# Nikhil-Doye/voice-enabled-browser-automation

Measured on AMD Instinct MI355X. Metric: voice-to-intent p50 latency (ms) + ASR RTF; 10s utterance; Llama-3-8B brain, lower is better.
Workload: dtype bf16; 1 GPU; model=whisper-tiny + llama3-8b, global_batch=1, parallelism=dp1, budget_chars=512, hipgraph=True

## Files before the change

### csrc/bindings.cpp

```cpp
#include <mutex>
#include <string>

#include <torch/extension.h>
#include <ATen/hip/impl/HIPStreamMasqueradingAsCUDA.h>
#include <c10/core/DeviceGuard.h>

#include "kernels/vwa_kernels.h"

namespace {

using at::Tensor;
using OptTensor = c10::optional<Tensor>;
constexpr auto kBF16 = at::kBFloat16;
constexpr auto kF8 = at::kFloat8_e4m3fn;

hipStream_t cur_stream(const Tensor& t) {
  return c10::hip::getCurrentHIPStreamMasqueradingAsCUDA(t.device().index()).stream();
}

const uint16_t* bfp(const Tensor& t) { return reinterpret_cast<const uint16_t*>(t.data_ptr()); }
uint16_t* bfp_mut(const Tensor& t) { return reinterpret_cast<uint16_t*>(t.data_ptr()); }
const uint16_t* bfp_opt(const OptTensor& t) { return t.has_value() ? bfp(*t) : nullptr; }
uint16_t* bfp_mut_opt(const OptTensor& t) { return t.has_value() ? bfp_mut(*t) : nullptr; }
template <class T>
// ... 570 lines not shown

int chain_grid(const Tensor& a) {
  const char* e = std::getenv("VWA_CHAIN_GRID_DIV");
  const int div = e ? std::atoi(e) : 1, cus = device_cus(a);
  return div > 1 ? cus / div : cus;
}

void chain_schedule(ChainParams& cp) {
  cp.pre2 = 1;
  cp.next0 = 1;
  cp.xdma = 1;
  cp.osub = 1;
  cp.lds_item_req = 1;
  cp.lds_item2_req = 1;
  cp.attn_flag = 1;
  cp.xfirst = 1;
  cp.xwait = 1;
  cp.o_nt2 = 1;
  cp.d_nt2 = 1;
  cp.pre_mask = 8;
  cp.qkv_flags = 0;
  cp.kv_prefetch = 0;
  cp.attn_pre = 0;
  if (const char* e = std::getenv("VWA_CHAIN_SCHED")) {
    std::string s(e);
    size_t at = 0;
    while (at < s.size()) {
      const size_t comma = s.find(',', at), eq = s.find('=', at);
      const size_t end = comma == std::string::npos ? s.size() : comma;
      if (eq != std::string::npos && eq < end) {
        const std::string k = s.substr(at, eq - at);
        const int v = std::atoi(s.substr(eq + 1, end - eq - 1).c_str());
        if (k == "pre2") cp.pre2 = v;
        else if (k == "next0") cp.next0 = v;
        else if (k == "xdma") cp.xdma = v;
        else if (k == "osub") cp.osub = v;
        else if (k == "lds1") cp.lds_item_req = v;
        else if (k == "lds2") cp.lds_item2_req = v;
        else if (k == "aflag") cp.attn_flag = v;
        else if (k == "pre_mask") cp.pre_mask = v;
        else if (k == "pre_waves") cp.pre_waves = v;
        else if (k == "xfirst") cp.xfirst = v;
        else if (k == "xwait") cp.xwait = v;
        else if (k == "xw_late") cp.xw_late = v;
        else if (k == "poll_free") cp.poll_free = v;
        else if (k == "o_nt2") cp.o_nt2 = v;
        else if (k == "d_nt2") cp.d_nt2 = v;
        else if (k == "qkv_flags") cp.qkv_flags = v;
        else if (k == "kv_pf") cp.kv_prefetch = v;
        else if (k == "attn_pre") cp.attn_pre = v;
      }
      at = end + 1;
    }
  }
}

void set_resid(SkinnyParams& p, const Tensor& h) {
  p.Y = h.data_ptr();
  p.ldy = (int)h.stride(0);
  p.R = bfp(h);
  p.ldr = (int)h.stride(0);
}

void set_chain_sync(ChainParams& cp, const Tensor& a, const Tensor& bar, const Tensor& work, int64_t bar_mode) {
  check_vec(bar, a, at::kInt, 384, "bar");
  TORCH_CHECK(aligned(bar, 128), "bar must be 128-byte aligned");
  check_vec(work, a, at::kInt, 8192 + 4096 + 1, "work");
  cp.bar = reinterpret_cast<unsigned*>(bar.data_ptr<int>());
  cp.bar_mode = (int)bar_mode;
  cp.tickets = reinterpret_cast<unsigned*>(work.data_ptr<int>());
  cp.max_tiles = 8192;
  cp.part = reinterpret_cast<float*>(work.data_ptr<int>() + 8192);
  cp.part_floats = (int)(work.numel() - 8192);
// ... 84 lines not shown
                            n_kv_heads, head_dim, a_scale, a_n_splits, *a_part_o, *a_part_ml, *a_counters, att);
    TORCH_CHECK(a_n_splits > 1, "attention phase: the in-launch chunk merge needs n_splits > 1");
    cp.attn_g = (int)(n_q_heads / n_kv_heads);
    TORCH_CHECK(a_row_table.has_value(), "attention phase: a_row_table (per-row block tables) is required");
    TORCH_CHECK(a_block_size == 16, "attention phase: 16-token KV blocks (mq_attention.h FINE addressing)");
    const Tensor& rtab = *a_row_table;
    check_vec(rtab, h, at::kInt, 0, "a_row_table");
    TORCH_CHECK(rtab.dim() == 2 && rtab.size(0) >= M && rtab.size(1) <= 128 && rtab.size(1) % 2 == 0,
                "a_row_table must be int32 [>= rows, <= 128 (even)] contiguous");
    cp.attn.row_table = rtab.data_ptr<int>();
    cp.attn.rt_stride = (int)rtab.size(1);
    if (a_plan_mode) {
      TORCH_CHECK(a_plan_mode == 1 || a_plan_mode == 2, "a_plan_mode: 1 write, 2 read");
      TORCH_CHECK(a_plan.has_value(), "a_plan_mode needs a_plan");
      check_vec(*a_plan, h, at::kInt, (int64_t)chain_grid(h) * 16, "a_plan");
      cp.attn.plan = a_plan->data_ptr<int>();
      cp.attn.plan_mode = (int)a_plan_mode;
    }
  }
  int64_t lds = 0;
  Tensor desc = chain_upload(cp, h, lds);
  if (!desc.numel()) return {desc, 0};
  return {desc, lds | (cp.n >= 3 && cp.ph[2].xg ? (int64_t)1 << 24 : 0) | (cp.d_nt2 ? (int64_t)1 << 27 : 0) |
                    (s_o.has_value() ? (int64_t)1 << 25 : 0) | (cp.o_nt2 ? (int64_t)1 << 26 : 0)};
}

std::tuple<Tensor, int64_t> chain_make_seq(int64_t seq, std::vector<Tensor> X, std::vector<Tensor> W,
                                           std::vector<OptTensor> bias, std::vector<OptTensor> ln_c,
                                           std::vector<Tensor> Y, std::vector<int64_t> epi, double eps, int64_t n_heads,
                                           int64_t head_dim, OptTensor positions, OptTensor slots, OptTensor k_cache,
                                           OptTensor v_cache, Tensor bar, Tensor work, int64_t bar_mode, bool w_tiled) {
  const size_t n = X.size();
  TORCH_CHECK(n >= 2 && n <= (size_t)kChainMaxPhases && W.size() == n && bias.size() == n && ln_c.size() == n &&
                  Y.size() == n && epi.size() == n,
              "chain_make_seq: one X/W/bias/ln_c/Y/epi per phase");
  TORCH_CHECK(seq == 1 || seq == 2, "chain_make_seq: seq 1 (Whisper tail) or 2 (Whisper middle)");
  const Tensor& a = X[0];
  c10::DeviceGuard g(a.device());
  check_anchor(a, "X");
  ChainParams cp{};
  set_chain_sync(cp, a, bar, work, bar_mode);
  for (size_t i = 0; i < n; ++i) {
    check_gpu(X[i], a, kBF16, "X");
    SkinnyParams& p = cp.ph[i].p;
    p = base_params(X[i], "X", W[i], "W", bias[i], "bias", false, eps, c10::nullopt, w_tiled);
    cp.ph[i].epi = (int)epi[i];
// ... 556 lines not shown
```

### csrc/kernels/mq_attention.h

```cpp
#pragma once
#include "common.h"
#include "vwa_kernels.h"

namespace {
using namespace vwa;

typedef __attribute__((address_space(1))) const int gint;
VWA_DEVICE int64_t kv_offset(const KVView& kv, int seq, int kvh, int t) {
  const int blk = *(gint*)(kv.block_table + (int64_t)seq * kv.table_stride + t / kv.block_size);
  return (int64_t)blk * kv.stride_block + (int64_t)kvh * kv.stride_head + (int64_t)(t % kv.block_size) * kv.stride_tok;
}

VWA_DEVICE __amdgpu_buffer_rsrc_t rsrc_f32(float* p, int64_t n) {
  return __builtin_amdgcn_make_buffer_rsrc(p, (short)0, (int)(n * 4), 0x00020000);
}
VWA_DEVICE void st_sc1_f2(__amdgpu_buffer_rsrc_t r, int64_t idx, float a, float b) {
  __builtin_amdgcn_raw_buffer_store_b64(__builtin_bit_cast(u32x2, make_float2(a, b)), r, (int)(idx * 4), 0, 16);
}
VWA_DEVICE void st_sc1_f1(__amdgpu_buffer_rsrc_t r, int64_t idx, float a) {
  __builtin_amdgcn_raw_buffer_store_b32(__float_as_uint(a), r, (int)(idx * 4), 0, 16);
}
VWA_DEVICE float2 ld_sc1_f2(__amdgpu_buffer_rsrc_t r, int64_t idx) {
  return __builtin_bit_cast(float2, __builtin_amdgcn_raw_buffer_load_b64(r, (int)(idx * 4), 0, 16));
}
// ... 36 lines not shown
    __hip_atomic_store(gp(reinterpret_cast<unsigned long long*>(dst) + 1), (unsigned long long)v.z | ((unsigned long long)v.w << 32),
                       __ATOMIC_RELAXED, __HIP_MEMORY_SCOPE_AGENT);
  } else {
    *gp(reinterpret_cast<u32x4*>(dst)) = u32x4{v.x, v.y, v.z, v.w};
  }
}

template <int D, int NW>
struct MqLds {
  static constexpr int OWP = D + 4;
  static constexpr int vimg = 0;
  static constexpr int ow = NW * kMqStep * 256;
  static constexpr int mlw = ow + NW * kMqCols * OWP * 4;
  static constexpr int last = mlw + NW * kMqCols * 2 * 4;
  static constexpr int bytes = last + 16;
};

struct NoIdle {
  VWA_DEVICE void operator()() const {}
};
struct NoStamp {
  VWA_DEVICE void operator()(int) const {}
};

template <int D, int G, int NW, bool SC1OUT, bool DB = true, bool FINE = false, class OnIdle = NoIdle,
          class Stamp = NoStamp, class OnKv = NoIdle>
VWA_DEVICE bool mq_body(const DecodeAttnParams& p, unsigned char* lds, int grid, int bid, OnIdle on_idle = {},
                        int* n_items_out = nullptr, Stamp stamp = {}, unsigned long long* done = nullptr,
                        int* n_final_out = nullptr, OnKv on_kv = {}) {
  constexpr int kWv = NW;
  constexpr int kChunk = FINE ? kMqStep : NW * kMqStep;
  constexpr int RG = kMqCols / G;
  constexpr int NKS = D / 32;
  constexpr int NDT = D / 16;
  constexpr int NCH = D / 8;
  constexpr int NVL = kMqStep * NCH / 64;
  constexpr int OWP = D + 4;
  using L = MqLds<D, NW>;
  float* ow = reinterpret_cast<float*>(lds + L::ow);
  float* mlw = reinterpret_cast<float*>(lds + L::mlw);
  int& s_last = *reinterpret_cast<int*>(lds + L::last);

  const int nkv = p.n_kv_heads, nq = p.n_q_heads;
  const int lane = VWA_TX & 63, w = VWA_TX >> 6;
  const int n = lane & 15, g = lane >> 4;

  constexpr bool rowtab = FINE;
  const __amdgpu_buffer_rsrc_t r_rt = __builtin_amdgcn_make_buffer_rsrc(
      const_cast<int*>(p.row_table), (short)0, rowtab ? p.rows * p.rt_stride * 4 : 0, 0x00020000);
  int* s_meta = reinterpret_cast<int*>(lds + L::vimg);
  int2 rt[4];
  int ev = 0;
  bool plan = false;
  if constexpr (FINE) {
    if (p.plan_mode == 2) {
      const __amdgpu_buffer_rsrc_t r_pl = __builtin_amdgcn_make_buffer_rsrc(p.plan, (short)0, (bid + 1) * 64, 0x00020000);
      ev = (int)__builtin_amdgcn_raw_buffer_load_b32(r_pl, (bid * 16 + (lane & 15)) * 4, 0, 16);
#pragma unroll
      for (int r = 0; r < 4; ++r)
        rt[r] = __builtin_bit_cast(int2, __builtin_amdgcn_raw_buffer_load_b64(
                                             r_rt, 2 * lane < p.rt_stride ? (r * p.rt_stride + 2 * lane) * 4 : 0x7FFFFFF0, 0, 0));
      plan = __builtin_amdgcn_readlane(ev, 2) != 3 && __builtin_amdgcn_readlane(ev, 10) == p.rows;
    }
  }
  if (w == 0 && !plan) {
#pragma unroll
    for (int r = 0; r < 4; ++r)
      *reinterpret_cast<int2*>(s_meta + r * 128 + 2 * lane) = __builtin_bit_cast(
          int2, __builtin_amdgcn_raw_buffer_load_b64(
                    r_rt, 2 * lane < p.rt_stride ? (r * p.rt_stride + 2 * lane) * 4 : 0x7FFFFFF0, 0, 0));
    const __amdgpu_buffer_rsrc_t r_sid =
        __builtin_amdgcn_make_buffer_rsrc(const_cast<int*>(p.seq_ids), (short)0, p.rows * 4, 0x00020000);
    const __amdgpu_buffer_rsrc_t r_ctx =
        __builtin_amdgcn_make_buffer_rsrc(const_cast<int*>(p.ctx_lens), (short)0, p.rows * 4, 0x00020000);
    s_meta[512 + lane] = (int)__builtin_amdgcn_raw_buffer_load_b32(r_sid, lane * 4, 0, 0);
    s_meta[576 + lane] = (int)__builtin_amdgcn_raw_buffer_load_b32(r_ctx, lane * 4, 0, 0);
    if constexpr (!FINE) {
      const __amdgpu_buffer_rsrc_t r_sh =
// ... 19 lines not shown
  }
  const bool cascade = !FINE && P > 0 && n_real > 0 && p.n_splits > RG;
  unsigned long long run_starts = seq_starts;
  if (cascade) {
    const unsigned long long real = n_real >= 64 ? ~0ull : ((1ull << n_real) - 1ull);
    run_starts = 1ull | (n_real < p.rows ? (1ull << n_real) : 0ull) | (seq_starts & ~real);
  }
  const int run0 = 63 - __builtin_clzll(run_starts & ((2ull << lane) - 1ull));
  const unsigned long long leaders = __ballot(lane < p.rows && (lane - run0) % RG == 0);
  const int n_groups = __builtin_popcountll(leaders);
  const int my_rank = __builtin_popcountll(leaders & ((1ull << lane) - 1ull));
  static_assert(!FINE || NW == 8, "the FINE merge pairs two threads per (column, slice): 512 threads");
  const int tgt = FINE ? grid : max(1, grid / 2);
  const int n_pc = cascade ? max(1, min(p.n_splits - RG, tgt / max(1, n_groups * nkv) - RG)) : 0;
  const int n_eff = cascade ? n_pc + RG : max(1, min(FINE ? min(p.n_splits, 16) : p.n_splits, tgt / max(1, n_groups * nkv)));
  const int n_items = plan ? __builtin_amdgcn_readlane(ev, 0) : n_groups * nkv * n_eff;
  if (n_items_out) *n_items_out = n_items;
  if (n_final_out) *n_final_out = plan ? __builtin_amdgcn_readlane(ev, 1) : n_groups * nkv;
  stamp(17);
  const bool multi = n_items > grid;
  auto write_plan = [&](int st, int kvh, int r0, int nr, int kbeg, int kend, int nact, int slot, int c) {
    if (!FINE || p.plan_mode != 1 || w != 0) return;
    const int cr = __shfl(c, lane & 3, 64);
    const int i = lane & 15;
    const int v = i == 0 ? n_items : i == 1 ? n_groups * nkv : i == 2 ? (multi ? 3 : st) : i == 3 ? kvh : i == 4 ? r0
                : i == 5 ? nr : i == 6 ? kbeg : i == 7 ? kend : i == 8 ? nact : i == 9 ? slot : i == 10 ? p.rows
                : i == 11 ? 0 : cr;
    if (lane < 16) p.plan[bid * 16 + i] = v;
  };
  if (bid >= n_items) {
    write_plan(0, 0, 0, 0, 0, 0, 0, 0, 0);
    on_idle();
    return true;
  }

  auto publish = [&]() {
    if (done == nullptr) return;
    asm volatile("s_waitcnt vmcnt(0)" ::: "memory");
    __syncthreads();
    if (VWA_TX == 0) __hip_atomic_fetch_add(gp(done), 1ull, __ATOMIC_RELAXED, __HIP_MEMORY_SCOPE_AGENT);
  };
  for (int item = bid; item < n_items; item += grid) {
  if (item == bid) stamp(18);
  int kvh, r0, nr, CL, kbeg, kend, nact, slot, kv_seq, ctx_n;
  const int rho = n / G;
  if (plan) {
    if (__builtin_amdgcn_readlane(ev, 2) != 1) continue;
    kvh = __builtin_amdgcn_readlane(ev, 3);
    r0 = __builtin_amdgcn_readlane(ev, 4);
    nr = __builtin_amdgcn_readlane(ev, 5);
// ... 85 lines not shown
  auto make_qf = [&]() {
    const float qs = p.scale * 1.4426950408889634f;
    const int64_t qo = (int64_t)(r0 + min(rho, nr - 1)) * p.ldq + (kvh * G + n % G) * D + 8 * g;
    const __amdgpu_buffer_rsrc_t r_q = __builtin_amdgcn_make_buffer_rsrc(
        const_cast<u16*>(p.q), (short)0, FINE ? (int)((int64_t)p.rows * p.ldq * 2) : 0, 0x00020000);
#pragma unroll
    for (int ks = 0; ks < NKS; ++ks) {
      float f[8];
      if constexpr (FINE) {
        const u32x4 v = __builtin_amdgcn_raw_buffer_load_b128(r_q, (int)((qo + 32 * ks) * 2), 0, 16);
        unpack8(make_uint4(v.x, v.y, v.z, v.w), f);
      } else {
        unpack8(ld128(p.q + qo + 32 * ks), f);
      }
#pragma unroll
      for (int j = 0; j < 8; ++j) f[j] = rho < nr ? f[j] * qs : 0.f;
      qf[ks] = as_bf16x8(pack8(f));
    }
  };
  if constexpr (DB) {
    make_qf();
    if (item == bid) stamp(10);
  }
  const int2 rtr = r0 == 0 ? rt[0] : r0 == 1 ? rt[1] : r0 == 2 ? rt[2] : rt[3];

  auto load_step = [&](int kb, uint4 (&kr)[2][NKS], uint4 (&vr)[NVL]) {
    int64_t ko[2], vo[NVL];
    auto offsets = [&](auto off) {
#pragma unroll
      for (int t = 0; t < 2; ++t) ko[t] = off(min(kb + 8 * (n >> 2) + 4 * t + (n & 3), kmax));
#pragma unroll
      for (int i = 0; i < NVL; ++i) vo[i] = off(min(kb + (i * 64 + lane) / NCH, kmax));
    };
    if constexpr (rowtab) {
      const int tl = kb >> 5;
      const int64_t bA = (int64_t)__builtin_amdgcn_readlane(rtr.x, tl) * p.kv.stride_block,
                    bB = (int64_t)__builtin_amdgcn_readlane(rtr.y, tl) * p.kv.stride_block;
      const int64_t hoff = (int64_t)kvh * p.kv.stride_head;
      const int st = (int)p.kv.stride_tok;
      offsets([&](int key) -> int64_t { return ((key & 16) ? bB : bA) + hoff + (key & 15) * st; });
    } else {
      offsets([&](int key) -> int64_t { return kv_offset(p.kv, kv_seq, kvh, key); });
    }
#pragma unroll
    for (int t = 0; t < 2; ++t)
#pragma unroll
      for (int ks = 0; ks < NKS; ++ks) kr[t][ks] = ld128(p.kv.k + ko[t] + 8 * g + 32 * ks);
#pragma unroll
    for (int i = 0; i < NVL; ++i) vr[i] = ld128(p.kv.v + vo[i] + 8 * ((i * 64 + lane) % NCH));
  };

  float m_run = -INFINITY, l_run = 0.f;
  f32x4 o[NDT];
#pragma unroll
  for (int dt = 0; dt < NDT; ++dt) o[dt] = f32x4{0.f, 0.f, 0.f, 0.f};
  unsigned char* vi = lds + L::vimg + w * kMqStep * 256;
  if (item == bid) stamp(21);

  auto compute_step = [&](int kb, const uint4 (&kr)[2][NKS], const uint4 (&vr)[NVL]) {
#pragma unroll
    for (int i = 0; i < NVL; ++i) {
      const int idx = i * 64 + lane;
      *reinterpret_cast<uint4*>(vi + vimg_off(idx / NCH, idx % NCH)) = vr[i];
    }
    f32x4 s[2];
#pragma unroll
    for (int t = 0; t < 2; ++t) {
      s[t] = f32x4{0.f, 0.f, 0.f, 0.f};
#pragma unroll
      for (int ks = 0; ks < NKS; ++ks) s[t] = mfma16(as_bf16x8(kr[t][ks]), qf[ks], s[t]);
    }
    float pv[8];
    float mx = -INFINITY;
#pragma unroll
    for (int t = 0; t < 2; ++t)
#pragma unroll
      for (int i = 0; i < 4; ++i) {
        const float v = (kb + 8 * g + 4 * t + i < ctx_n) ? s[t][i] : -INFINITY;
        pv[4 * t + i] = v;
        mx = fmaxf(mx, v);
      }
    mx = fmaxf(mx, __shfl_xor(mx, 16, 64));
    mx = fmaxf(mx, __shfl_xor(mx, 32, 64));
    const float m_new = fmaxf(m_run, mx);
    const float alpha = (m_run == -INFINITY) ? 0.f : exp2f(m_run - m_new);
    float ps = 0.f;
#pragma unroll
    for (int j = 0; j < 8; ++j) {
      pv[j] = (pv[j] == -INFINITY) ? 0.f : exp2f(pv[j] - m_new);
      ps += pv[j];
    }
    l_run = l_run * alpha + ps;
    m_run = m_new;
    const bf16x8 pb = as_bf16x8(pack8(pv));
    const int q4 = n >> 2, p4 = n & 3;
#pragma unroll
    for (int dt = 0; dt < NDT; ++dt) {
      const int ch = 2 * dt + (p4 >> 1), sub = 8 * (p4 & 1);
      const uint2 lo = lds_tr16(vi + vimg_off(8 * g + q4, ch) + sub);
      const uint2 hi = lds_tr16(vi + vimg_off(8 * g + 4 + q4, ch) + sub);
      o[dt] = mfma16(as_bf16x8(make_uint4(lo.x, lo.y, hi.x, hi.y)), pb, o[dt] * alpha);
    }
  };

  if constexpr (DB) {
    if (nsteps > 0) {
      uint4 kA[2][NKS], vA[NVL], kB[2][NKS], vB[NVL];
      load_step(wb, kA, vA);
      for (int s = 0; s < nsteps; s += 2) {
        if (s + 1 < nsteps) load_step(wb + (s + 1) * kMqStep, kB, vB);
        compute_step(wb + s * kMqStep, kA, vA);
        if (s + 1 >= nsteps) break;
        if (s + 2 < nsteps) load_step(wb + (s + 2) * kMqStep, kA, vA);
        compute_step(wb + (s + 1) * kMqStep, kB, vB);
      }
    }
  } else {
    bool have_q = false;
    for (int s = FINE ? w : 0; s < nsteps; s += FINE ? kWv : 1) {
      uint4 kA[2][NKS], vA[NVL];
      if (item == bid && s == w) stamp(13);
      load_step(wb + s * kMqStep, kA, vA);
      if (!have_q) {
        make_qf();
        have_q = true;
      }
      if (item == bid && s == w) stamp(15);
      compute_step(wb + s * kMqStep, kA, vA);
    }
    if (item == bid) on_kv();
  }

  float l_tot = l_run + __shfl_xor(l_run, 16, 64);
  l_tot += __shfl_xor(l_tot, 32, 64);
  if (g == 0) {
    mlw[(w * kMqCols + n) * 2 + 0] = m_run;
    mlw[(w * kMqCols + n) * 2 + 1] = l_tot;
  }
#pragma unroll
  for (int dt = 0; dt < NDT; ++dt)
    *reinterpret_cast<float4*>(&ow[(w * kMqCols + n) * OWP + 16 * dt + 4 * g]) = make_float4(o[dt][0], o[dt][1], o[dt][2], o[dt][3]);
  __syncthreads();

  const int cn = VWA_TX >> 4, dc = VWA_TX & 15;
  const int crow = r0 + cn / G, ch = kvh * G + cn % G;
  const bool act = cn / G < nr && dc < NCH;
  const __amdgpu_buffer_rsrc_t r_o = rsrc_f32(p.part_o, (int64_t)p.rows * p.n_splits * nq * D);
  const __amdgpu_buffer_rsrc_t r_ml = rsrc_f32(p.part_ml, (int64_t)p.rows * p.n_splits * nq * 2);
  float acc[8];
  if (act) {
    float M = -INFINITY;
// ... 131 lines not shown
```

### csrc/kernels/skinny_stream.hip

```cpp
#include "common.h"
#include "vwa_kernels.h"
#include "mq_attention.h"

using namespace vwa;

namespace {

enum Epi { EPI_STORE = 0, EPI_RESID = 1, EPI_SWIGLU = 2, EPI_GELU = 3, EPI_QKV = 4 };

constexpr unsigned kOOB = 0xFFFFFFF0u;

VWA_DEVICE uint4 bload(__amdgpu_buffer_rsrc_t r, unsigned off) {
  u32x4 v = __builtin_amdgcn_raw_buffer_load_b128(r, (int)off, 0, 0);
  return make_uint4(v.x, v.y, v.z, v.w);
}
template <int AUX>
VWA_DEVICE uint4 bload_w(__amdgpu_buffer_rsrc_t r, unsigned off) {
  u32x4 v = __builtin_amdgcn_raw_buffer_load_b128(r, (int)off, 0, AUX);
  return make_uint4(v.x, v.y, v.z, v.w);
}
constexpr unsigned kOOB2 = 0x80000000u;
template <int AUX>
VWA_DEVICE uint4 bload_w_so(__amdgpu_buffer_rsrc_t r, unsigned voff, int soff) {
  u32x4 v = __builtin_amdgcn_raw_buffer_load_b128(r, (int)voff, soff, AUX);
// ... 1059 lines not shown
                                          : (I == 0 ? EPI_RESID : EPI_STORE);
};

VWA_DEVICE int qkv_group(const SkinnyParams& q, int tile) {
  const int head = tile * 16 / q.head_dim, G = q.n_q_heads / q.n_kv_heads;
  return head < q.n_q_heads ? head / G : head < q.n_q_heads + q.n_kv_heads ? head - q.n_q_heads
                                                                            : head - q.n_q_heads - q.n_kv_heads;
}
VWA_DEVICE long long qkv_tiles_per_group(const SkinnyParams& q) {
  return (long long)(q.n_q_heads / q.n_kv_heads + 2) * q.head_dim / 16;
}

template <int KS>
VWA_DEVICE void qkv_signal(const ChainPhase& ph, unsigned long long* bar) {
  asm volatile("s_waitcnt vmcnt(0)" ::: "memory");
  lds_sync();
  const PhaseRange r = chain_range<KS>(ph);
  if (VWA_TX == 0)
    for (int it = 0; it < r.n_items; ++it)
      __hip_atomic_fetch_add(gp(&bar[kBarQkv + kBarQkvStride * qkv_group(ph.p, r.u0 + it)]), 1ull, __ATOMIC_RELAXED,
                             __HIP_MEMORY_SCOPE_AGENT);
}

VWA_DEVICE void qkv_wait(unsigned long long* bar, const unsigned long long* base, unsigned long long add, int g0, int g1) {
  if (VWA_TX < 64) {
    for (int g = g0; g < g1; ++g) {
      const unsigned long long tgt = base[g] + add;
      const unsigned long long* w = &bar[kBarQkv + kBarQkvStride * g];
      int spins = 0;
      while (true) {
        unsigned long long v;
        asm volatile("s_load_dwordx2 %0, %1, 0x0 glc\n\ts_waitcnt lgkmcnt(0)" : "=s"(v) : "s"(w) : "memory");
        if ((long long)(v - tgt) >= 0) break;
        __builtin_amdgcn_s_sleep(1);
        if (++spins > kChainSpinLimit) {
          if (VWA_TX == 0) __hip_atomic_store(gp(&bar[kBarErr]), 1ull, __ATOMIC_RELAXED, __HIP_MEMORY_SCOPE_AGENT);
          break;
        }
      }
    }
  }
  lds_sync();
}

VWA_DEVICE void kv_prefetch(const DecodeAttnParams& a, int ev, unsigned char* lds) {
  const int kvh = __builtin_amdgcn_readlane(ev, 3), r0 = __builtin_amdgcn_readlane(ev, 4);
  const int kbeg = __builtin_amdgcn_readlane(ev, 6), kend = __builtin_amdgcn_readlane(ev, 7);
  const int c0 = __builtin_amdgcn_readlane(ev, 12);
  const int nk = min(min(kend, c0 - 1) - kbeg, 128);
// ... 17 lines not shown
    if (512 * i + w * 64 >= nk * 16) break;
    const long long e = (long long)blk[i] * a.kv.stride_block + (long long)kvh * a.kv.stride_head +
                        (long long)(key & 15) * a.kv.stride_tok;
    const unsigned off = q < nk * 16 ? (unsigned)(e * 2 + (q & 15) * 16) : 0x7FFFFFF0u;
    __builtin_amdgcn_raw_ptr_buffer_load_lds(rk, dst, 16, off, 0, 0, 0);
    __builtin_amdgcn_raw_ptr_buffer_load_lds(rv, dst, 16, off, 0, 0, 0);
  }
}

template <int KS, int SEQ, int NPH, int AG, int WA, bool XG2 = false, bool F8 = false, bool O2 = false, bool D2 = false,
          bool MULTI = false>
__global__ __launch_bounds__(KS * 64) void chain_kernel(const ChainParams* __restrict__ cpp, int n_layers) {
  extern __shared__ __attribute__((aligned(16))) char smem[];
  static_assert(!MULTI || (SEQ == 0 && NPH == 4 && AG > 0 && !XG2), "multi-layer launch: Llama tails with attention");
  const int nwg = (int)gridDim.x;
  unsigned long long* bar = reinterpret_cast<unsigned long long*>(cpp->bar);
  unsigned long long bar_next = chain_base(bar, nwg, cpp->bar_mode);
  const bool tpr = cpp->tp.world > 1;
  const int e0 = tpr ? __hip_atomic_load(gp(cpp->tp.epoch), __ATOMIC_RELAXED, __HIP_MEMORY_SCOPE_AGENT) : 0;
  unsigned long long qkv_base[8] = {};
  const bool qsig = MULTI && cpp->qkv_flags && cpp->bar_mode == 2 && cpp->ph[3].nb == 1 &&
                    cpp->ph[3].p.n_kv_heads <= 8 && cpp->attn_flag;
  if constexpr (MULTI) {
    if (qsig && VWA_TX < 64) {
      const unsigned long long tpg = (unsigned long long)qkv_tiles_per_group(cpp->ph[3].p);
      for (int g = 0; g < cpp->ph[3].p.n_kv_heads; ++g) {
        const unsigned long long v = __hip_atomic_load(gp(&bar[kBarQkv + kBarQkvStride * g]), __ATOMIC_RELAXED, __HIP_MEMORY_SCOPE_AGENT);
        qkv_base[g] = v / tpg * tpg;
      }
    }
  }
  bool pf_prev = false, pf_next = false;
  for (int li = 0; li < (MULTI ? n_layers : 1); ++li) {
  pf_prev = pf_next;
  pf_next = false;
  const ChainParams& cp = cpp[li];
  static_assert(sizeof(ChainParams) <= 25 * 64, "descriptor warm-up covers 25 lines");
  {
    unsigned junk;
    asm("s_load_dword %0, %1, 0x0\n\t""s_load_dword %0, %1, 0x40\n\t""s_load_dword %0, %1, 0x80\n\t""s_load_dword %0, %1, 0xc0\n\t"
        "s_load_dword %0, %1, 0x100\n\t""s_load_dword %0, %1, 0x140\n\t""s_load_dword %0, %1, 0x180\n\t""s_load_dword %0, %1, 0x1c0\n\t"
        "s_load_dword %0, %1, 0x200\n\t""s_load_dword %0, %1, 0x240\n\t""s_load_dword %0, %1, 0x280\n\t""s_load_dword %0, %1, 0x2c0\n\t"
        "s_load_dword %0, %1, 0x300\n\t""s_load_dword %0, %1, 0x340\n\t""s_load_dword %0, %1, 0x380\n\t""s_load_dword %0, %1, 0x3c0\n\t"
        "s_load_dword %0, %1, 0x400\n\t""s_load_dword %0, %1, 0x440\n\t""s_load_dword %0, %1, 0x480\n\t""s_load_dword %0, %1, 0x4c0\n\t""s_load_dword %0, %1, 0x500\n\t"
        "s_load_dword %0, %1, 0x540\n\t""s_load_dword %0, %1, 0x580\n\t""s_load_dword %0, %1, 0x5c0\n\t""s_load_dword %0, %1, 0x600\n\t"
        "s_waitcnt lgkmcnt(0)"
        : "=&s"(junk)
        : "s"(cpp + li));
    if (junk == 0x9e3779b9u) __builtin_amdgcn_s_sleep(1);
  }
  uint4 A[ChainShape<KS, F8>::R] = {}, B[ChainShape<KS, F8>::R] = {};
  unsigned long long gen;
  const int er = e0 + 2 * li;
  int nts = 0;
  auto stamp = [&]() {
    if (cp.ts && VWA_TX == 0) *gp(cp.ts + blockIdx.x * kTsStride + nts) = __builtin_amdgcn_s_memrealtime();
    ++nts;
  };
  stamp();
  constexpr int E0 = SeqEpi<SEQ, 0>::value, E1 = SeqEpi<SEQ, 1>::value, E2 = SeqEpi<SEQ, 2>::value,
                E3 = SeqEpi<SEQ, 3>::value;
  int pre0 = cp.pre2;
  int ob0 = 0, on = 0;
  bool nx = false;
  bool apre = false;
  auto setup0 = [&](int n_attn) {
    const bool sub = cp.osub && n_attn > 0 && n_attn <= nwg / 2;
    ob0 = sub ? n_attn : 0;
    on = sub ? nwg - n_attn : 0;
    nx = cp.next0 && chain_range<KS>(cp.ph[0], ob0, on).n_items <= 1;
  };
  auto issue0 = [&](int pre) {
    if (nx) {
      chain_issue_item<E0, KS, WA, false, F8, O2>(cp.ph[0], B, 0, ob0, on);
      chain_issue_item<E1, KS, WA, false, F8>(cp.ph[1], A, 0);
    } else {
      chain_issue_first<E0, KS, WA, false, F8, O2>(cp.ph[0], B, A, pre, ob0, on);
    }
  };
  auto preload1 = [&]() {
    chain_preload<PhaseShape<E1, KS, false, F8>::NT, PhaseShape<E1, KS, false, F8>::U, WA, F8>(
        cp.ph[1].p, cp.ph[1].nb, chain_range<KS>(cp.ph[1]), 2, smem + cp.lds_item);
  };
  if constexpr (AG > 0) {
   if (cp.attn_flag) {
    int n_attn = 0, n_final = 0;
    unsigned long long* done = &bar[kBarAttnDone];
    const bool idle = mq_body<128, AG, KS, true, false, true>(cp.attn, reinterpret_cast<unsigned char*>(smem), nwg,
                                                        (int)blockIdx.x, [&]() {
                                                          setup0(n_attn);
                                                          issue0(pre0);
                                                        }, &n_attn, [&](int k) {
                                                          if ((k == 15 || k == 10) && cp.ts) asm volatile("s_waitcnt vmcnt(0)" ::: "memory");
                                                          if (cp.ts && VWA_TX == 0)
                                                            *gp(cp.ts + blockIdx.x * kTsStride + k) = __builtin_amdgcn_s_memrealtime();
                                                        }, done, &n_final, [&]() {
                                                          if constexpr (F8) {
                                                            if (cp.attn_pre && cp.osub && n_attn > 0 && n_attn <= nwg / 2 &&
                                                                (int)blockIdx.x < n_attn) {
                                                              chain_issue_item<E1, KS, WA, false, F8>(cp.ph[1], A, 0);
                                                              apre = true;
                                                            }
                                                          }
                                                        });
    if (!idle) setup0(n_attn);
    stamp();
    if (MULTI && !idle && pf_prev) asm volatile("s_waitcnt vmcnt(0)" ::: "memory");
    lds_sync();
    if (!idle) {
      pre0 = 0;
      issue0(0);
    }
    if (cp.lds_item && (int)(VWA_TX >> 6) < cp.lds_item_waves) preload1();
    if (chain_range<KS>(cp.ph[0], ob0, on).n_items > 0) {
      if (VWA_TX < 64) {
        const unsigned long long tgt = (unsigned long long)n_final;
        int spins = 0;
        while (true) {
          unsigned long long v;
          asm volatile("s_load_dwordx2 %0, %1, 0x0 glc\n\ts_waitcnt lgkmcnt(0)" : "=s"(v) : "s"(done) : "memory");
          if (v >= tgt) break;
          __builtin_amdgcn_s_sleep(1);
          if (++spins > kChainSpinLimit) {
            if (VWA_TX == 0) __hip_atomic_store(gp(&bar[kBarErr]), 1ull, __ATOMIC_RELAXED, __HIP_MEMORY_SCOPE_AGENT);
            break;
          }
        }
// ... 57 lines not shown
    stamp();
    chain_phase<E2, KS, WA, XG2, F8, D2>(cp, 2, A, B, smem, preb_of(2), 0, 0, 0, prew || XG2);
    stamp();
    if (SEQ == 0 && tpr) {
      chain_tp_reduce(cp, 1, er + 2, bar, nwg, bar_next);
      if (blockIdx.x == 0 && VWA_TX == 0)
        __hip_atomic_store(gp(cp.tp.epoch), er + 2, __ATOMIC_RELAXED, __HIP_MEMORY_SCOPE_AGENT);
    }
  }
  if constexpr (NPH >= 4) {
   if (!MULTI || cp.n >= 4) {
    gen = chain_arrive(bar, nwg, cp.bar_mode, bar_next);
    if (!stg && prew) chain_issue_first<E3, KS, WA, false, F8>(cp.ph[3], A, B, preb_of(3));
    chain_wait(bar, gen, cp.bar_mode);
    stamp();
    chain_phase<E3, KS, WA, false, F8>(cp, 3, A, B, smem, preb_of(3), 0, 0, 0, prew);
    stamp();
   }
  }
  if constexpr (MULTI) {
    if (li + 1 < n_layers) {
      if (qsig) qkv_signal<KS>(cp.ph[3], bar);
      else gen = chain_arrive(bar, nwg, cp.bar_mode, bar_next);
      const DecodeAttnParams& na = cpp[li + 1].attn;
      int st = 3, ev = 0;
      if (cpp[li + 1].attn_flag && na.plan_mode == 2) {
        const __amdgpu_buffer_rsrc_t r_pl =
            __builtin_amdgcn_make_buffer_rsrc(na.plan, (short)0, ((int)blockIdx.x + 1) * 64, 0x00020000);
        ev = (int)__builtin_amdgcn_raw_buffer_load_b32(r_pl, ((int)blockIdx.x * 16 + (VWA_TX & 15)) * 4, 0, 16);
        st = __builtin_amdgcn_readlane(ev, 10) == na.rows ? __builtin_amdgcn_readlane(ev, 2) : 3;
      }
      if (st != 0 && st != 2) {
        if (st == 1 && cp.kv_prefetch) {
          kv_prefetch(na, ev, reinterpret_cast<unsigned char*>(smem));
          pf_next = true;
        }
        if (!qsig) {
          chain_wait(bar, gen, cp.bar_mode);
        } else {
          const int kvh = __builtin_amdgcn_readlane(ev, 3);
          const unsigned long long add = (unsigned long long)qkv_tiles_per_group(cp.ph[3].p) * (unsigned long long)(li + 1);
          if (st == 1) qkv_wait(bar, qkv_base, add, kvh, kvh + 1);
          else qkv_wait(bar, qkv_base, add, 0, cp.ph[3].p.n_kv_heads);
        }
      }
    }
  }
  }
}

}

extern "C" int vwa_chain_prepare(ChainParams* cp, int grid) {
  constexpr int KS = 8;
  constexpr int R = ChainShape<KS>::R;
  if (cp->n < 2 || cp->n > kChainMaxPhases || grid < 1) return -10;
  static const int kSeq[3][kChainMaxPhases] = {{EPI_RESID, EPI_SWIGLU, EPI_RESID, EPI_QKV},
                                               {EPI_RESID, EPI_GELU, EPI_RESID, EPI_QKV},
                                               {EPI_RESID, EPI_STORE, -1, -1}};
  if (cp->seq < 0 || cp->seq > 2 || (cp->seq == 2 ? cp->n != 2 : cp->n < (cp->seq == 0 ? 2 : 3))) return -10;
  if (cp->seq == 0 && cp->n == 2) return -10;
  size_t lds = 0;
  for (int i = 0; i < cp->n; ++i) {
    ChainPhase& ph = cp->ph[i];
    const SkinnyParams& p = ph.p;
    if (ph.epi != kSeq[cp->seq][i]) return -10;
    ph.nt = (ph.epi == EPI_SWIGLU) ? 2 : 1;
    if (i == 0 && cp->o_nt2) {
// ... 189 lines not shown
```

### csrc/kernels/vwa_kernels.h

```cpp
#pragma once
#include <hip/hip_runtime.h>
#include <stdint.h>

struct SkinnyParams {
  const uint16_t* X; int ldx;
  const uint16_t* W;
  int M, N, K;
  const uint16_t* bias;
  int fuse_rms; float eps;
  void* Y; int ldy; int y_f32;
  const uint16_t* R; int ldr;
  int n_q_heads, n_kv_heads, head_dim, use_rope;
  const int* positions;
  const int64_t* slots;
  const float* rope;
  uint16_t* q_out; int ldq;
  uint16_t* k_cache; uint16_t* v_cache;
  int block_size;
  int64_t cache_stride_block, cache_stride_head, cache_stride_tok;
  const float* w_scale;
  int w_first;
  const float* ln_c;
  int w_tiled;
  const uint32_t* col_mask; int col_mask_ld; int col_mask_rows;
// ... 53 lines not shown
  unsigned* tickets;
  int max_tiles;
  unsigned long long* ts;
  DecodeAttnParams attn;
  int attn_g;
  int lds_item;
  int lds_item_waves;
  int lds_item_req;
  int lds_item2;
  int lds_item2_waves;
  int lds_item2_req;
  int attn_flag;
  int pre_mask;
  int pre_waves;
  int xfirst;
  int xwait;
  int xw_late;
  int poll_free;
  int o_nt2;
  int d_nt2;
  int kv_prefetch;
  int qkv_flags;
  int attn_pre;
  ChainTP tp;
};

struct GemmParams {
  const uint16_t* X; int ldx;
  const uint16_t* W; int w_tiled;
  int M, N, K;
  void* Y; int ldy; int y_f32;
  const uint16_t* bias;
  const uint16_t* R; int ldr;
  const float* rstd;
  float* ws; int splits; int kg_per_split;
  const float* sx; const float* sw;
  int nbatch; int64_t bsx, bsy, bsr;
  int cus; int64_t ws_cap;
  int n_q_heads, n_kv_heads, head_dim, use_rope;
  const int* positions; const int64_t* slots; const float* rope;
  uint16_t* q_out; int ldq; uint16_t* k_cache; uint16_t* v_cache; int block_size;
  int64_t cache_sb, cache_sh, cache_st;
  unsigned long long* ss_out; unsigned long long* ss_zero; int ss_zero_n; const unsigned long long* ss_in;
  float ss_eps;
};

// ... 105 lines not shown
```

Baseline: 237.2 ms.

## Issue next-layer attention KV loads before the cross-layer barrier wait

Moves the inter-layer plan read and barrier wait to the start of each layer in the persistent multi-layer chain kernel. When enabled, it adds an early attention head that loads the first step's row table and K/V registers before waiting on the QKV barrier. The plan now records the first cached-prefix boundary, so only keys at or past that bound (newly written this layer) are reloaded after the wait. It also unrolls the QKV barrier wait and reads barrier bases with scalar loads. The cost is extra live registers and more complex correctness logic around which cached keys are stale, and the F8 attn_pre path is disabled for the multi-layer kernel.

```diff
diff --git a/csrc/bindings.cpp b/csrc/bindings.cpp
--- a/csrc/bindings.cpp
+++ b/csrc/bindings.cpp
@@ -616,6 +616,7 @@
   cp.qkv_flags = 0;
   cp.kv_prefetch = 0;
   cp.attn_pre = 0;
+  cp.attn_early = 1;
   if (const char* e = std::getenv("VWA_CHAIN_SCHED")) {
     std::string s(e);
     size_t at = 0;
@@ -643,6 +644,7 @@
         else if (k == "qkv_flags") cp.qkv_flags = v;
         else if (k == "kv_pf") cp.kv_prefetch = v;
         else if (k == "attn_pre") cp.attn_pre = v;
+        else if (k == "attn_early") cp.attn_early = v;
       }
       at = end + 1;
     }
@@ -773,6 +775,7 @@
   Tensor desc = chain_upload(cp, h, lds);
   if (!desc.numel()) return {desc, 0};
   return {desc, lds | (cp.n >= 3 && cp.ph[2].xg ? (int64_t)1 << 24 : 0) | (cp.d_nt2 ? (int64_t)1 << 27 : 0) |
+                    (cp.attn_early && cp.attn_g > 0 ? (int64_t)1 << 28 : 0) |
                     (s_o.has_value() ? (int64_t)1 << 25 : 0) | (cp.o_nt2 ? (int64_t)1 << 26 : 0)};
 }
 
diff --git a/csrc/kernels/mq_attention.h b/csrc/kernels/mq_attention.h
--- a/csrc/kernels/mq_attention.h
+++ b/csrc/kernels/mq_attention.h
@@ -82,12 +82,74 @@
 struct NoStamp {
   VWA_DEVICE void operator()(int) const {}
 };
+struct NoEarly {
+  static constexpr bool enabled = false;
+};
+
+template <int D>
+VWA_DEVICE void mq_step_offsets(const DecodeAttnParams& p, int2 rtr, int kvh, int kb, int klim, int64_t (&ko)[2],
+                                int64_t (&vo)[kMqStep * (D / 8) / 64]) {
+  constexpr int NCH = D / 8, NVL = kMqStep * NCH / 64;
+  const int lane = VWA_TX & 63, n = lane & 15;
+  const int tl = kb >> 5;
+  const int64_t bA = (int64_t)__builtin_amdgcn_readlane(rtr.x, tl) * p.kv.stride_block,
+                bB = (int64_t)__builtin_amdgcn_readlane(rtr.y, tl) * p.kv.stride_block;
+  const int64_t hoff = (int64_t)kvh * p.kv.stride_head;
+  const int st = (int)p.kv.stride_tok;
+  auto off = [&](int key) -> int64_t { return ((key & 16) ? bB : bA) + hoff + (key & 15) * st; };
+#pragma unroll
+  for (int t = 0; t < 2; ++t) ko[t] = off(min(kb + 8 * (n >> 2) + 4 * t + (n & 3), klim));
+#pragma unroll
+  for (int i = 0; i < NVL; ++i) vo[i] = off(min(kb + (i * 64 + lane) / NCH, klim));
+}
+
+template <int D>
+struct MqEarly {
+  static constexpr bool enabled = true;
+  static constexpr int NKS = D / 32, NVL = kMqStep * (D / 8) / 64;
+  int& on;
+  int& kv;
+  int& ev;
+  int& bound;
+  int2& rtr;
+  uint4 (&k)[2 * NKS];
+  uint4 (&v)[NVL];
+};
+
+template <int D>
+VWA_DEVICE void mq_head(const DecodeAttnParams& p, int ev, MqEarly<D> e) {
+  constexpr int NKS = D / 32, NCH = D / 8, NVL = kMqStep * NCH / 64;
+  const int lane = VWA_TX & 63, w = VWA_TX >> 6, g = lane >> 4;
+  const __amdgpu_buffer_rsrc_t r_rt =
+      __builtin_amdgcn_make_buffer_rsrc(const_cast<int*>(p.row_table), (short)0, p.rows * p.rt_stride * 4, 0x00020000);
+  const int kvh = __builtin_amdgcn_readlane(ev, 3), r0 = __builtin_amdgcn_readlane(ev, 4);
+  const int2 rtr = __builtin_bit_cast(int2, __builtin_amdgcn_raw_buffer_load_b64(
+                                                r_rt, 2 * lane < p.rt_stride ? (r0 * p.rt_stride + 2 * lane) * 4 : 0x7FFFFFF0, 0, 0));
+  e.rtr = rtr;
+  e.ev = ev;
+  e.on = 1;
+  const int kbeg = __builtin_amdgcn_readlane(ev, 6), kend = __builtin_amdgcn_readlane(ev, 7);
+  e.bound = __builtin_amdgcn_readlane(ev, 11) - 1;
+  const int kb = kbeg + w * kMqStep;
+  const int klim = min(kend, e.bound) - 1;
+  if (kb > klim) return;
+  int64_t ko[2], vo[NVL];
+  mq_step_offsets<D>(p, rtr, kvh, kb, klim, ko, vo);
+#pragma unroll
+  for (int t = 0; t < 2; ++t)
+#pragma unroll
+    for (int ks = 0; ks < NKS; ++ks) e.k[t * NKS + ks] = ld128(p.kv.k + ko[t] + 8 * g + 32 * ks);
+#pragma unroll
+  for (int i = 0; i < NVL; ++i) e.v[i] = ld128(p.kv.v + vo[i] + 8 * ((i * 64 + lane) % NCH));
+  e.kv = 1;
+}
 
 template <int D, int G, int NW, bool SC1OUT, bool DB = true, bool FINE = false, class OnIdle = NoIdle,
-          class Stamp = NoStamp, class OnKv = NoIdle>
+          class Stamp = NoStamp, class OnKv = NoIdle, class Early = NoEarly>
 VWA_DEVICE bool mq_body(const DecodeAttnParams& p, unsigned char* lds, int grid, int bid, OnIdle on_idle = {},
                         int* n_items_out = nullptr, Stamp stamp = {}, unsigned long long* done = nullptr,
-                        int* n_final_out = nullptr, OnKv on_kv = {}) {
+                        int* n_final_out = nullptr, OnKv on_kv = {}, Early early = {}) {
+  static_assert(!Early::enabled || (FINE && !DB), "the early head feeds the FINE single-register-set loop");
   constexpr int kWv = NW;
   constexpr int kChunk = FINE ? kMqStep : NW * kMqStep;
   constexpr int RG = kMqCols / G;
@@ -112,8 +174,13 @@
   int2 rt[4];
   int ev = 0;
   bool plan = false;
+  bool pre = false;
+  if constexpr (Early::enabled) pre = early.on != 0;
   if constexpr (FINE) {
-    if (p.plan_mode == 2) {
+    if (pre) {
+      if constexpr (Early::enabled) ev = early.ev;
+      plan = true;
+    } else if (p.plan_mode == 2) {
       const __amdgpu_buffer_rsrc_t r_pl = __builtin_amdgcn_make_buffer_rsrc(p.plan, (short)0, (bid + 1) * 64, 0x00020000);
       ev = (int)__builtin_amdgcn_raw_buffer_load_b32(r_pl, (bid * 16 + (lane & 15)) * 4, 0, 16);
 #pragma unroll
@@ -179,10 +246,13 @@
   auto write_plan = [&](int st, int kvh, int r0, int nr, int kbeg, int kend, int nact, int slot, int c) {
     if (!FINE || p.plan_mode != 1 || w != 0) return;
     const int cr = __shfl(c, lane & 3, 64);
+    int cf = (lane < p.rows && sl == __shfl(sl, min(r0, 63), 64)) ? cl : 0x7FFFFFFF;
+#pragma unroll
+    for (int o = 1; o < 64; o <<= 1) cf = min(cf, __shfl_xor(cf, o, 64));
     const int i = lane & 15;
     const int v = i == 0 ? n_items : i == 1 ? n_groups * nkv : i == 2 ? (multi ? 3 : st) : i == 3 ? kvh : i == 4 ? r0
                 : i == 5 ? nr : i == 6 ? kbeg : i == 7 ? kend : i == 8 ? nact : i == 9 ? slot : i == 10 ? p.rows
-                : i == 11 ? 0 : cr;
+                : i == 11 ? cf : cr;
     if (lane < 16) p.plan[bid * 16 + i] = v;
   };
   if (bid >= n_items) {
@@ -314,9 +384,11 @@
     make_qf();
     if (item == bid) stamp(10);
   }
-  const int2 rtr = r0 == 0 ? rt[0] : r0 == 1 ? rt[1] : r0 == 2 ? rt[2] : rt[3];
-
-  auto load_step = [&](int kb, uint4 (&kr)[2][NKS], uint4 (&vr)[NVL]) {
+  int2 rtr = r0 == 0 ? rt[0] : r0 == 1 ? rt[1] : r0 == 2 ? rt[2] : rt[3];
+  if constexpr (Early::enabled)
+    if (pre) rtr = early.rtr;
+
+  auto load_step = [&](int kb, uint4 (&kr)[2 * NKS], uint4 (&vr)[NVL]) {
     int64_t ko[2], vo[NVL];
     auto offsets = [&](auto off) {
 #pragma unroll
@@ -324,22 +396,41 @@
 #pragma unroll
       for (int i = 0; i < NVL; ++i) vo[i] = off(min(kb + (i * 64 + lane) / NCH, kmax));
     };
+    if constexpr (rowtab) {
+      mq_step_offsets<D>(p, rtr, kvh, kb, kmax, ko, vo);
+    } else {
+      offsets([&](int key) -> int64_t { return kv_offset(p.kv, kv_seq, kvh, key); });
+    }
+#pragma unroll
+    for (int t = 0; t < 2; ++t)
+#pragma unroll
+      for (int ks = 0; ks < NKS; ++ks) kr[t * NKS + ks] = ld128(p.kv.k + ko[t] + 8 * g + 32 * ks);
+#pragma unroll
+    for (int i = 0; i < NVL; ++i) vr[i] = ld128(p.kv.v + vo[i] + 8 * ((i * 64 + lane) % NCH));
+  };
+  auto reload_step = [&](int kb, int bound, uint4 (&kr)[2 * NKS], uint4 (&vr)[NVL]) {
     if constexpr (rowtab) {
       const int tl = kb >> 5;
       const int64_t bA = (int64_t)__builtin_amdgcn_readlane(rtr.x, tl) * p.kv.stride_block,
                     bB = (int64_t)__builtin_amdgcn_readlane(rtr.y, tl) * p.kv.stride_block;
       const int64_t hoff = (int64_t)kvh * p.kv.stride_head;
       const int st = (int)p.kv.stride_tok;
-      offsets([&](int key) -> int64_t { return ((key & 16) ? bB : bA) + hoff + (key & 15) * st; });
-    } else {
-      offsets([&](int key) -> int64_t { return kv_offset(p.kv, kv_seq, kvh, key); });
-    }
-#pragma unroll
-    for (int t = 0; t < 2; ++t)
-#pragma unroll
-      for (int ks = 0; ks < NKS; ++ks) kr[t][ks] = ld128(p.kv.k + ko[t] + 8 * g + 32 * ks);
-#pragma unroll
-    for (int i = 0; i < NVL; ++i) vr[i] = ld128(p.kv.v + vo[i] + 8 * ((i * 64 + lane) % NCH));
+      auto off = [&](int key) -> int64_t { return ((key & 16) ? bB : bA) + hoff + (key & 15) * st; };
+#pragma unroll
+      for (int t = 0; t < 2; ++t) {
+        const int key = min(kb + 8 * (n >> 2) + 4 * t + (n & 3), kmax);
+        if (key >= bound) {
+          const u16* src = p.kv.k + off(key) + 8 * g;
+#pragma unroll
+          for (int ks = 0; ks < NKS; ++ks) kr[t * NKS + ks] = ld128(src + 32 * ks);
+        }
+      }
+#pragma unroll
+      for (int i = 0; i < NVL; ++i) {
+        const int key = min(kb + (i * 64 + lane) / NCH, kmax);
+        if (key >= bound) vr[i] = ld128(p.kv.v + off(key) + 8 * ((i * 64 + lane) % NCH));
+      }
+    }
   };
 
   float m_run = -INFINITY, l_run = 0.f;
@@ -349,7 +440,7 @@
   unsigned char* vi = lds + L::vimg + w * kMqStep * 256;
   if (item == bid) stamp(21);
 
-  auto compute_step = [&](int kb, const uint4 (&kr)[2][NKS], const uint4 (&vr)[NVL]) {
+  auto compute_step = [&](int kb, const uint4 (&kr)[2 * NKS], const uint4 (&vr)[NVL]) {
 #pragma unroll
     for (int i = 0; i < NVL; ++i) {
       const int idx = i * 64 + lane;
@@ -360,7 +451,7 @@
     for (int t = 0; t < 2; ++t) {
       s[t] = f32x4{0.f, 0.f, 0.f, 0.f};
 #pragma unroll
-      for (int ks = 0; ks < NKS; ++ks) s[t] = mfma16(as_bf16x8(kr[t][ks]), qf[ks], s[t]);
+      for (int ks = 0; ks < NKS; ++ks) s[t] = mfma16(as_bf16x8(kr[t * NKS + ks]), qf[ks], s[t]);
     }
     float pv[8];
     float mx = -INFINITY;
@@ -397,7 +488,7 @@
 
   if constexpr (DB) {
     if (nsteps > 0) {
-      uint4 kA[2][NKS], vA[NVL], kB[2][NKS], vB[NVL];
+      uint4 kA[2 * NKS], vA[NVL], kB[2 * NKS], vB[NVL];
       load_step(wb, kA, vA);
       for (int s = 0; s < nsteps; s += 2) {
         if (s + 1 < nsteps) load_step(wb + (s + 1) * kMqStep, kB, vB);
@@ -409,16 +500,32 @@
     }
   } else {
     bool have_q = false;
-    for (int s = FINE ? w : 0; s < nsteps; s += FINE ? kWv : 1) {
-      uint4 kA[2][NKS], vA[NVL];
-      if (item == bid && s == w) stamp(13);
-      load_step(wb + s * kMqStep, kA, vA);
-      if (!have_q) {
-        make_qf();
-        have_q = true;
-      }
-      if (item == bid && s == w) stamp(15);
-      compute_step(wb + s * kMqStep, kA, vA);
+    auto key_steps = [&](uint4 (&kA)[2 * NKS], uint4 (&vA)[NVL]) {
+      for (int s = FINE ? w : 0; s < nsteps; s += FINE ? kWv : 1) {
+        if (item == bid && s == w) stamp(13);
+        bool carried = false;
+        if constexpr (Early::enabled) carried = pre && early.kv != 0 && s == w;
+        if (carried) {
+          if constexpr (Early::enabled)
+            if (min(wb + s * kMqStep + kMqStep - 1, kmax) >= early.bound)
+              reload_step(wb + s * kMqStep, early.bound, kA, vA);
+        } else {
+          load_step(wb + s * kMqStep, kA, vA);
+        }
+        if (!have_q) {
+          make_qf();
+          have_q = true;
+        }
+        if (item == bid && s == w) stamp(15);
+        compute_step(wb + s * kMqStep, kA, vA);
+        if (item == bid && s == w) stamp(59);
+      }
+    };
+    if constexpr (Early::enabled) {
+      key_steps(early.k, early.v);
+    } else {
+      uint4 kA[2 * NKS], vA[NVL];
+      key_steps(kA, vA);
     }
     if (item == bid) on_kv();
   }
diff --git a/csrc/kernels/skinny_stream.hip b/csrc/kernels/skinny_stream.hip
--- a/csrc/kernels/skinny_stream.hip
+++ b/csrc/kernels/skinny_stream.hip
@@ -1105,9 +1105,11 @@
                              __HIP_MEMORY_SCOPE_AGENT);
 }
 
-VWA_DEVICE void qkv_wait(unsigned long long* bar, const unsigned long long* base, unsigned long long add, int g0, int g1) {
+VWA_DEVICE void qkv_wait(unsigned long long* bar, const unsigned long long (&base)[8], unsigned long long add, int g0, int g1) {
   if (VWA_TX < 64) {
-    for (int g = g0; g < g1; ++g) {
+#pragma unroll
+    for (int g = 0; g < 8; ++g) {
+      if (g < g0 || g >= g1) continue;
       const unsigned long long tgt = base[g] + add;
       const unsigned long long* w = &bar[kBarQkv + kBarQkvStride * g];
       int spins = 0;
@@ -1171,18 +1173,23 @@
   const bool qsig = MULTI && cpp->qkv_flags && cpp->bar_mode == 2 && cpp->ph[3].nb == 1 &&
                     cpp->ph[3].p.n_kv_heads <= 8 && cpp->attn_flag;
   if constexpr (MULTI) {
-    if (qsig && VWA_TX < 64) {
+    if (qsig) {
       const unsigned long long tpg = (unsigned long long)qkv_tiles_per_group(cpp->ph[3].p);
-      for (int g = 0; g < cpp->ph[3].p.n_kv_heads; ++g) {
-        const unsigned long long v = __hip_atomic_load(gp(&bar[kBarQkv + kBarQkvStride * g]), __ATOMIC_RELAXED, __HIP_MEMORY_SCOPE_AGENT);
-        qkv_base[g] = v / tpg * tpg;
-      }
-    }
-  }
-  bool pf_prev = false, pf_next = false;
+#pragma unroll
+      for (int g = 0; g < 8; ++g)
+        if (g < cpp->ph[3].p.n_kv_heads) {
+          unsigned long long v;
+          asm volatile("s_load_dwordx2 %0, %1, 0x0 glc\n\ts_waitcnt lgkmcnt(0)"
+                       : "=s"(v)
+                       : "s"(&bar[kBarQkv + kBarQkvStride * g])
+                       : "memory");
+          qkv_base[g] = v / tpg * tpg;
+        }
+    }
+  }
+  unsigned long long gen = 0;
   for (int li = 0; li < (MULTI ? n_layers : 1); ++li) {
-  pf_prev = pf_next;
-  pf_next = false;
+  bool pf_prev = false;
   const ChainParams& cp = cpp[li];
   static_assert(sizeof(ChainParams) <= 25 * 64, "descriptor warm-up covers 25 lines");
   {
@@ -1199,7 +1206,6 @@
     if (junk == 0x9e3779b9u) __builtin_amdgcn_s_sleep(1);
   }
   uint4 A[ChainShape<KS, F8>::R] = {}, B[ChainShape<KS, F8>::R] = {};
-  unsigned long long gen;
   const int er = e0 + 2 * li;
   int nts = 0;
   auto stamp = [&]() {
@@ -1207,6 +1213,44 @@
     ++nts;
   };
   stamp();
+  int e_on = 0, e_kv = 0, e_ev = 0, e_bound = 0;
+  int2 e_rt = make_int2(0, 0);
+  uint4 e_k[2 * MqEarly<128>::NKS] = {}, e_v[MqEarly<128>::NVL] = {};
+  const MqEarly<128> early{e_on, e_kv, e_ev, e_bound, e_rt, e_k, e_v};
+  if constexpr (MULTI) {
+    if (li > 0) {
+      const ChainParams& pp = cpp[li - 1];
+      const DecodeAttnParams& na = cp.attn;
+      auto tstamp = [&](int k) {
+        if (cp.ts && VWA_TX == 0) *gp(cp.ts + blockIdx.x * kTsStride + k) = __builtin_amdgcn_s_memrealtime();
+      };
+      int st = 3, ev = 0;
+      if (cp.attn_flag && na.plan_mode == 2) {
+        const __amdgpu_buffer_rsrc_t r_pl =
+            __builtin_amdgcn_make_buffer_rsrc(na.plan, (short)0, ((int)blockIdx.x + 1) * 64, 0x00020000);
+        ev = (int)__builtin_amdgcn_raw_buffer_load_b32(r_pl, ((int)blockIdx.x * 16 + (VWA_TX & 15)) * 4, 0, 16);
+        st = __builtin_amdgcn_readlane(ev, 10) == na.rows ? __builtin_amdgcn_readlane(ev, 2) : 3;
+      }
+      if (st != 0 && st != 2) {
+        if (st == 1 && cp.attn_early) {
+          mq_head<128>(na, ev, early);
+          tstamp(57);
+        } else if (st == 1 && pp.kv_prefetch) {
+          kv_prefetch(na, ev, reinterpret_cast<unsigned char*>(smem));
+          pf_prev = true;
+        }
+        if (!qsig) {
+          chain_wait(bar, gen, pp.bar_mode);
+        } else {
+          const int kvh = __builtin_amdgcn_readlane(ev, 3);
+          const unsigned long long add = (unsigned long long)qkv_tiles_per_group(pp.ph[3].p) * (unsigned long long)li;
+          if (st == 1) qkv_wait(bar, qkv_base, add, kvh, kvh + 1);
+          else qkv_wait(bar, qkv_base, add, 0, pp.ph[3].p.n_kv_heads);
+        }
+        tstamp(58);
+      }
+    }
+  }
   constexpr int E0 = SeqEpi<SEQ, 0>::value, E1 = SeqEpi<SEQ, 1>::value, E2 = SeqEpi<SEQ, 2>::value,
                 E3 = SeqEpi<SEQ, 3>::value;
   int pre0 = cp.pre2;
@@ -1244,14 +1288,14 @@
                                                           if (cp.ts && VWA_TX == 0)
                                                             *gp(cp.ts + blockIdx.x * kTsStride + k) = __builtin_amdgcn_s_memrealtime();
                                                         }, done, &n_final, [&]() {
-                                                          if constexpr (F8) {
+                                                          if constexpr (F8 && !MULTI) {
                                                             if (cp.attn_pre && cp.osub && n_attn > 0 && n_attn <= nwg / 2 &&
                                                                 (int)blockIdx.x < n_attn) {
                                                               chain_issue_item<E1, KS, WA, false, F8>(cp.ph[1], A, 0);
                                                               apre = true;
                                                             }
                                                           }
-                                                        });
+                                                        }, early);
     if (!idle) setup0(n_attn);
     stamp();
     if (MULTI && !idle && pf_prev) asm volatile("s_waitcnt vmcnt(0)" ::: "memory");
@@ -1355,28 +1399,6 @@
     if (li + 1 < n_layers) {
       if (qsig) qkv_signal<KS>(cp.ph[3], bar);
       else gen = chain_arrive(bar, nwg, cp.bar_mode, bar_next);
-      const DecodeAttnParams& na = cpp[li + 1].attn;
-      int st = 3, ev = 0;
-      if (cpp[li + 1].attn_flag && na.plan_mode == 2) {
-        const __amdgpu_buffer_rsrc_t r_pl =
-            __builtin_amdgcn_make_buffer_rsrc(na.plan, (short)0, ((int)blockIdx.x + 1) * 64, 0x00020000);
-        ev = (int)__builtin_amdgcn_raw_buffer_load_b32(r_pl, ((int)blockIdx.x * 16 + (VWA_TX & 15)) * 4, 0, 16);
-        st = __builtin_amdgcn_readlane(ev, 10) == na.rows ? __builtin_amdgcn_readlane(ev, 2) : 3;
-      }
-      if (st != 0 && st != 2) {
-        if (st == 1 && cp.kv_prefetch) {
-          kv_prefetch(na, ev, reinterpret_cast<unsigned char*>(smem));
-          pf_next = true;
-        }
-        if (!qsig) {
-          chain_wait(bar, gen, cp.bar_mode);
-        } else {
-          const int kvh = __builtin_amdgcn_readlane(ev, 3);
-          const unsigned long long add = (unsigned long long)qkv_tiles_per_group(cp.ph[3].p) * (unsigned long long)(li + 1);
-          if (st == 1) qkv_wait(bar, qkv_base, add, kvh, kvh + 1);
-          else qkv_wait(bar, qkv_base, add, 0, cp.ph[3].p.n_kv_heads);
-        }
-      }
     }
   }
   }
diff --git a/csrc/kernels/vwa_kernels.h b/csrc/kernels/vwa_kernels.h
--- a/csrc/kernels/vwa_kernels.h
+++ b/csrc/kernels/vwa_kernels.h
@@ -99,6 +99,7 @@
   int kv_prefetch;
   int qkv_flags;
   int attn_pre;
+  int attn_early;
   ChainTP tp;
 };
 
```

Measured after the change: 237.4 ms. Within noise of the previous version (+0.1%).
